# celliern/triflow

Measured on AMD Instinct MI355X. Metric: implicit time-steps/s, 1e6-node 3-var system (member-steps/s over all GPUs), higher is better.
Workload: dtype f64; 1 GPU; BASELINE config 3: M3_film, N=1000000 nodes, periodic, fixed dt=0.001, ROS2; members_per_gpu=1, parallelism=ensemble members sharded by rank, no data-path collective

## Files before the change

__graft_entry__.py:

```python
import os
import sys

ROOT = os.path.dirname(os.path.abspath(__file__))
if ROOT not in sys.path:
    sys.path.insert(0, ROOT)

PREBUILT = ["M1_advdiff", "M2_diff", "M3_film", "M5_stiff"]


def build():
    from triflow_amd import compilers, workloads
    from triflow_amd.model import Model
    compilers.build_runtime_library()
    for name in PREBUILT:
        model = Model(*workloads.model_args(name), hold_compilation=True)
        for seg in (4, 8):
            compilers.build_code_object(model, 0, seg=seg)
    import triflow_amd


def smoke():
    import numpy as np
    from triflow_amd import Model, schemes, workloads
    from oracle import numpy_path as ora
    name, fd, pars, dt, _ = workloads.config_inputs(3, 4096)
    model = Model(*workloads.model_args(name))
    ref = Model(*workloads.model_args(name), compiler=ora.numpy_compiler)
    F = model.F(model.fields_template(**fd), pars)
    Fo = ref.F(ref.fields_template(**fd), pars)
    assert np.array_equal(F, Fo), "F differs from the oracle"
    J = model.J(model.fields_template(**fd), pars)
    Jo = ref.J(ref.fields_template(**fd), pars)
    assert abs(J - Jo).max() <= 4 * np.spacing(abs(Jo).max()), "J differs from the oracle"
    _, new = schemes.ROS2(model)(0.0, model.fields_template(**fd), dt, pars)
    _, new_o = ora.ROS2(ref)(0.0, ref.fields_template(**fd), dt, pars)
    err = np.abs(new.uflat - new_o.uflat).max() / np.abs(new_o.uflat).max()
    assert err < 1e-9, "ROS2 step differs from the oracle: %g" % err
    print("smoke ok: F bit-exact, J <= 4 ulp, ROS2 step rel err %.1e on %s (N=4096)" % (err, name))


if __name__ == "__main__":
    build()
```

triflow_amd/codegen.py:

```python

import ast
import hashlib
import inspect

import numpy as np
from sympy import lambdify

_FUNCS_1 = {"sqrt": "sqrt", "exp": "exp", "log": "log", "sin": "sin", "cos": "cos",
            "tan": "tan", "tanh": "tanh", "sinh": "sinh", "cosh": "cosh",
            "arctan": "atan", "arcsin": "asin", "arccos": "acos",
            "abs": "tf_abs", "absolute": "tf_abs", "fabs": "tf_abs", "sign": "tf_sign",
            "log10": "log10", "log2": "log2", "cbrt": "cbrt", "expm1": "expm1",
            "log1p": "log1p", "floor": "floor", "ceil": "ceil"}


class UnsupportedExpression(NotImplementedError):
    pass


def _dbl(value):
    f = float(value)
    if f != value and not isinstance(value, float):
        raise UnsupportedExpression("integer constant %r is not a double" % (value,))
    if f == int(f) and abs(f) < 2 ** 53:
        return "%d.0" % int(f)
    return f.hex()


class _CEmitter(ast.NodeVisitor):

    def __init__(self, names, uniform_names=()):
        self.names = names
        self.uniform_names = set(uniform_names)
        self.denominators = {}
        self.den_count = {}
        self.shared = {}
        self.host_consts = {}

    def host_const(self, node):
        src = ast.unparse(node)
        k = self.host_consts.setdefault(src, len(self.host_consts))
        return "tf_hc[%d]" % k

    def is_uniform(self, node):
        if isinstance(node, ast.Constant):
            return True
        if isinstance(node, ast.Name):
            return node.id in self.uniform_names or node.id in ("pi", "E", "e")
        if isinstance(node, ast.UnaryOp):
            return self.is_uniform(node.operand)
        if isinstance(node, ast.BinOp):
            return self.is_uniform(node.left) and self.is_uniform(node.right)
        if isinstance(node, ast.Call):
            args = []
            for a in node.args:
                args.extend(a.elts if isinstance(a, (ast.List, ast.Tuple)) else [a])
# ... 85 lines not shown
            for item in items[1:]:
                out = "%s(%s, %s)" % (fn, out, item)
            return out
        if name in ("maximum", "minimum"):
            fn = "tf_max" if name == "maximum" else "tf_min"
            return "%s(%s, %s)" % (fn, self.visit(node.args[0]), self.visit(node.args[1]))
        if name in _FUNCS_1 and len(node.args) == 1:
            if self.is_uniform(node.args[0]) and not isinstance(node.args[0], ast.Constant) \
                    and name not in ("abs", "absolute", "fabs", "sign", "floor", "ceil", "sqrt"):
                return self.host_const(node)
            return "%s(%s)" % (_FUNCS_1[name], self.visit(node.args[0]))
        raise UnsupportedExpression("function %r is not supported by the HIP compiler" % name)

    def generic_visit(self, node):
        raise UnsupportedExpression(ast.dump(node))


def _printed_expressions(symbolic_args, exprs):
    if not exprs:
        return []
    func = lambdify(symbolic_args, exprs, modules=[{"Heaviside": lambda *a: 1}, "numpy"],
                    cse=False)
    src = inspect.getsource(func)
    tree = ast.parse(src)
    fdef = tree.body[0]
    ret = fdef.body[-1]
    if len(fdef.body) != 1 or not isinstance(ret, ast.Return) \
            or not isinstance(ret.value, (ast.List, ast.Tuple)):
        raise UnsupportedExpression("unexpected lambdify output:\n" + src)
    return list(ret.value.elts)


def _c_ident(name):
    return "v_" + "".join(ch if ch.isalnum() else "_" for ch in name)


def _stencil_names(fields, pars, mp, parvec_mask):
    names = {}
    decls = []
    for f, name in enumerate(fields):
        for off in range(-mp, mp + 1):
            key = name if off == 0 else "%s_%s%d" % (name, "m" if off < 0 else "p", abs(off))
            names[key] = _c_ident(key)
            decls.append("const double %s = w[%d][%d];" % (_c_ident(key), f, off + mp))
    for k, name in enumerate(pars):
        names[name] = _c_ident(name)
        decls.append("const double %s = par[%d];" % (_c_ident(name), k))
    names["dx"] = "dx"
    names["x"] = "xc"
    uniform = {"dx"} | {name for k, name in enumerate(pars) if not (parvec_mask >> k) & 1}
    return names, decls, uniform


def lower_model(model, parvec_mask=0, seg=8, sweep_block=64):
    nvar = model._nvar
    fields = list(model._dep_vars) + list(model._help_funcs)
    nh = len(model._help_funcs)
    pars = list(model._pars)
    lo, hi = model._bounds
    mp = (model._window_range - 1) // 2
    if -lo != hi or hi != mp:
        raise UnsupportedExpression("asymmetric stencil window %r" % (model._bounds,))
    if mp < 1:
        mp = 1
    if nvar + nh > 16 or len(pars) > 16:
        raise UnsupportedExpression("too many fields / parameters for the HIP skeleton")
    if mp * nvar > 16:
        raise UnsupportedExpression(
            "the banded solver of the HIP back end handles b = (stencil half width) x (number of dependent "
            "variables) <= 16; this model has b = %d x %d = %d" % (mp, nvar, mp * nvar))
    sparse = [int(k) for k in model._sparse_indices[0]]
    nnz = len(sparse)
    real_mp = (model._window_range - 1) // 2
    pat_eq = [k % nvar for k in sparse]
    pat_var = [(k // nvar) % nvar for k in sparse]
    pat_off = [(k // nvar) // nvar - real_mp for k in sparse]

    names, decls, uniform = _stencil_names(fields, pars, mp, parvec_mask)
    f_nodes = _printed_expressions(model._symbolic_args, model.F_array.tolist())
    j_nodes = _printed_expressions(model._symbolic_args, model._J_sparse_array.tolist())
    host_consts = {}

    def emit_all(nodes):
        first = _CEmitter(names, uniform)
        for n in nodes:
            first.visit(n)
        second = _CEmitter(names, uniform)
        second.shared = first.den_count
        second.host_consts = host_consts
        return second, [second.visit(n) for n in nodes]

    emit_f, f_c = emit_all(f_nodes)
    emit_j, j_c = emit_all(j_nodes)
    uses_x = any("xc" in _tokens(s) for s in f_c + j_c + list(emit_f.denominators) + list(emit_j.denominators))

    j_uniform = [1 if emit_j.is_uniform(n) else 0 for n in j_nodes]

    j_alias, j_alias_scale = _proportional_entries(model, j_uniform)

    def body(outname, exprs, emitter, only=None):
        lines = ["    " + d for d in decls if only is None or d.split("=")[1].strip().startswith("par[")]
        lines += ["    const double* tf_hc = par + %d;" % len(pars)]
        lines += ["    (void)dx; (void)xc; (void)par; (void)tf_hc;"]
        for den, k in sorted(emitter.denominators.items(), key=lambda kv: kv[1]) if only is None else ():
            lines += ["    const double tf_den%d = %s;" % (k, den),
                      "    const double tf_rden%d = 1.0 / tf_den%d;" % (k, k)]
        lines += ["    %s[%d] = %s;" % (outname, i, e) for i, e in enumerate(exprs)
                  if only is None or only[i]]
        return "\n".join(lines)

    def arr(name, values, ctype="int"):
        vals = ", ".join(str(v) for v in values) if values else "0"
        return "static constexpr %s %s[%d] = {%s};" % (ctype, name, max(len(values), 1), vals)

    hc_list = [src_ for src_, _ in sorted(host_consts.items(), key=lambda kv: kv[1])]
    par_is_vec = [1 if (parvec_mask >> k) & 1 else 0 for k in range(len(pars))] + [0] * len(hc_list)
    if len(pars) + len(hc_list) > 16:
        raise UnsupportedExpression("too many parameters + host constants for the HIP skeleton")
    src = "\n".join([
        "// generated by triflow_amd.codegen -- do not edit",
        "// equations: " + " ; ".join(str(e) for e in model._diff_eqs),
        "#define TF_NVAR %d" % nvar,
        "#define TF_NH %d" % nh,
        "#define TF_MP %d" % mp,
        "#define TF_NNZ %d" % nnz,
        "#define TF_NPAR %d" % (len(pars) + len(host_consts)),
        "#define TF_SEG %d" % seg,
        "#define TF_SWEEP_BLOCK %d" % sweep_block,
        "#define TF_USES_X %d" % (1 if uses_x else 0),
        arr("tf_pat_eq", pat_eq), arr("tf_pat_var", pat_var), arr("tf_pat_off", pat_off),
        arr("tf_par_is_vec", par_is_vec, "bool"),
        arr("tf_j_uniform", j_uniform, "bool"),
        arr("tf_j_alias", j_alias), arr("tf_j_alias_scale", [_dbl(v) for v in j_alias_scale], "double"),
        "TF_DEVICE void tf_eval_F(const double (&w)[TF_NVAR + TF_NH][2 * TF_MP + 1], "
        "const double* par, double dx, double xc, double* F) {",
        body("F", f_c, emit_f),
        "}",
        "TF_DEVICE void tf_eval_J(const double (&w)[TF_NVAR + TF_NH][2 * TF_MP + 1], "
        "const double* par, double dx, double xc, double* J) {",
        body("J", j_c, emit_j),
        "}",
        "// the node-independent entries only (tf_j_uniform); same expressions, same bits",
        "TF_DEVICE void tf_eval_J_uniform(const double* par, double dx, double* J) {",
        "    const double xc = 0.0;",
        body("J", j_c, emit_j, only=j_uniform),
        "}",
        ""])
    spec = dict(nvar=nvar, nh=nh, npar=len(pars) + len(hc_list), npar_model=len(pars),
                host_consts=hc_list, mp=mp, nnz=nnz, seg=seg,
                sweep_block=sweep_block, uses_x=int(uses_x), parvec_mask=int(parvec_mask),
                b2=mp * nvar, pat_eq=pat_eq, pat_var=pat_var, pat_off=pat_off, j_uniform=j_uniform,
                j_alias=j_alias, j_alias_scale=j_alias_scale,
                fields=fields, pars=pars)
    return src, spec


PROBE_REDUCTIONS = ("sum", "mean", "integral", "max", "min", "argmax", "argmin")


def _lower_node_expressions(model, exprs, parvec_mask):
    fields = list(model._dep_vars) + list(model._help_funcs)
    pars = list(model._pars)
    mp = max((model._window_range - 1) // 2, 1)
    names, decls, uniform = _stencil_names(fields, pars, mp, parvec_mask)
    import sympy
    for e in exprs:
        if sympy.sympify(e).has(sympy.Heaviside):
            raise UnsupportedExpression("function 'Heaviside' is not supported in a probe or recorder: the HIP "
                                        "compiler takes it as identically one, as the reference does in J; "
                                        "write the step with Max / Min / sign")
    nodes = _printed_expressions(model._symbolic_args, list(exprs))
    first = _CEmitter(names, uniform)
    for n in nodes:
        first.visit(n)
    emit = _CEmitter(names, uniform)
    emit.shared = first.den_count
    out = [emit.visit(n) for n in nodes]
    hc_list = [src_ for src_, _ in sorted(emit.host_consts.items(), key=lambda kv: kv[1])]
    uses_x = any("xc" in _tokens(c) for c in out + list(emit.denominators))
    lines = ["    " + d for d in decls]
    lines += ["    (void)dx; (void)xc; (void)par; (void)tf_hc;"]
    for den, k in sorted(emit.denominators.items(), key=lambda kv: kv[1]):
        lines += ["    const double tf_den%d = %s;" % (k, den),
                  "    const double tf_rden%d = 1.0 / tf_den%d;" % (k, k)]
    return lines, out, hc_list, uses_x, pars


def lower_probes(model, exprs, reductions, parvec_mask=0):
    kinds = [PROBE_REDUCTIONS.index(r) for r in reductions]
    lines, out, hc_list, uses_x, pars = _lower_node_expressions(model, exprs, parvec_mask)
    lines += ["    P[%d] = %s;" % (i, c) for i, c in enumerate(out)]
    block = "\n".join([
        "// device probes, generated by triflow_amd.codegen.lower_probes -- do not edit",
        "// " + " ; ".join("%s: %s" % (r, e) for r, e in zip(reductions, exprs)),
        "#define TF_NPROBE %d" % len(out),
        "#define TF_NPROBE_HC %d" % len(hc_list),
        "#define TF_PROBE_USES_X %d" % (1 if uses_x else 0),
        "static constexpr int tf_probe_kind[%d] = {%s};" % (max(len(kinds), 1),
                                                           ", ".join(map(str, kinds)) or "0"),
        "TF_DEVICE void tf_eval_probe(const double (&w)[TF_NVAR + TF_NH][2 * TF_MP + 1], "
        "const double* par, const double* tf_hc, double dx, double xc, double* P) {",
        "\n".join(lines),
        "}",
        ""])
    spec = dict(nprobe=len(out), kinds=kinds, host_consts=hc_list, pars=pars, uses_x=int(uses_x))
    return block, spec
# ... 169 lines not shown
```

triflow_amd/csrc/tf_kernels.h:

```cpp
#pragma once
#include "tf_args.h"

#ifndef TF_DEVICE
#error "define TF_DEVICE (e.g. __device__ __forceinline__) before including tf_kernels.h"
#endif

#define TF_W (2 * TF_MP + 1)
#define TF_NF (TF_NVAR + TF_NH)
#define TF_B2 (TF_MP * TF_NVAR)

#include "tf_math.h"

#if defined(TF_STAMPS) && defined(__HIP_DEVICE_COMPILE__)
#define TF_STAMP(a, i) do { if ((a).stamps && blockIdx.x == gridDim.x / 2 && threadIdx.x == 0) \
        (a).stamps[i] = __builtin_amdgcn_s_memtime(); } while (0)
#define TF_STAMP_T(a, i, tid) do { if ((a).stamps && blockIdx.x == gridDim.x / 2 && blockIdx.y == 0 && threadIdx.x == (tid)) \
        (a).stamps[i] = __builtin_amdgcn_s_memtime(); } while (0)
#define TF_STAMP_REAL(a, i) do { if ((a).stamps && blockIdx.x == gridDim.x / 2 && threadIdx.x == 0) \
        (a).stamps[i] = __builtin_amdgcn_s_memrealtime(); } while (0)
#define TF_STAMP_IF(a, i, cond) do { if ((a).stamps && (cond) && threadIdx.x == 0) (a).stamps[i] = __builtin_amdgcn_s_memtime(); } while (0)
#define TF_STAMP_REAL_IF(a, i, cond) do { if ((a).stamps && (cond) && threadIdx.x == 0) (a).stamps[i] = __builtin_amdgcn_s_memrealtime(); } while (0)
#define TF_COUNT(a, i) do { if ((a).stamps && (threadIdx.x & 63) == 0) atomicAdd(&(a).stamps[i], 1ull); } while (0)
#define TF_STAMP_L1(a, dir, i) do { if ((dir) > 0 && blockIdx.y == 0) TF_STAMP(a, i); } while (0)
#define TF_WGTRACE(a, k, which) do { if ((a).stamps && threadIdx.x == 0 && blockIdx.y * gridDim.x + blockIdx.x < 1024) \
// ... 437 lines not shown
        const int64_t i = q / L.P, p = q - i * L.P;
        const int64_t s = (int64_t)v * L.plane + i * L.Ptot + (int64_t)e * L.P + p;
        const double d = a.a[s] - a.b[s];
        if (a.ord == 2) acc = tf_fma(d, d, acc);
        else { const double m = tf_abs(d); acc = (m > acc || m != m) ? m : acc; }
    }
    return acc;
}

TF_DEVICE void tfk_dirichlet_elem(const TfDirichletArgs& a, int t) {
    const TfLayout& L = a.L;
    if (t >= a.n * L.nsys) return;
    const int k = t % a.n, e = t / a.n;
    int g = a.node[k];
    if (g < 0) g += L.N;
    int p, i;
    tf_locate(L, g, p, i);
    a.fields[(int64_t)a.var[k] * L.plane + tf_idx(L, e * L.P + p, i)] = a.value[k];
}

TF_DEVICE void tfk_poke_elem(const TfPokeArgs& a, int t) {
    const TfLayout& L = a.L;
    if (t >= a.n * L.nsys) return;
    const int k = t % a.n, e = t / a.n;
    int g = 0, v = 0;
    double val = 0.0;
#pragma unroll
    for (int q = 0; q < TF_POKE_MAX; ++q)
        if (q == k) { g = a.node[q]; v = a.var[q]; val = a.value[q]; }
    if (g < 0) g += L.N;
    int p, i;
    tf_locate(L, g, p, i);
    a.fields[(int64_t)v * L.plane + tf_idx(L, e * L.P + p, i)] = val;
}


template <int B> struct TfBlk { double v[B][B]; };
template <int V> struct TfInt { static constexpr int value = V; };

template <int B>
TF_DEVICE void tf_blk_zero(double (&a)[B][B]) {
#pragma unroll
    for (int r = 0; r < B; ++r)
#pragma unroll
        for (int c = 0; c < B; ++c) a[r][c] = 0.0;
}
template <int B>
TF_DEVICE void tf_blk_copy(double (&d)[B][B], const double (&s)[B][B]) {
#pragma unroll
    for (int r = 0; r < B; ++r)
#pragma unroll
        for (int c = 0; c < B; ++c) d[r][c] = s[r][c];
}
template <int B>
TF_DEVICE void tf_mm_sub(double (&C)[B][B], const double (&A)[B][B], const double (&Bm)[B][B]) {
#pragma unroll
    for (int r = 0; r < B; ++r)
#pragma unroll
        for (int c = 0; c < B; ++c) {
            double acc = C[r][c];
#pragma unroll
            for (int k = 0; k < B; ++k) acc = tf_fma(-A[r][k], Bm[k][c], acc);
            C[r][c] = acc;
        }
}
template <int B>
TF_DEVICE void tf_mm(double (&C)[B][B], const double (&A)[B][B], const double (&Bm)[B][B]) {
#pragma unroll
    for (int r = 0; r < B; ++r)
#pragma unroll
        for (int c = 0; c < B; ++c) {
            double acc = 0.0;
#pragma unroll
            for (int k = 0; k < B; ++k) acc = tf_fma(A[r][k], Bm[k][c], acc);
            C[r][c] = acc;
        }
}
template <int B>
TF_DEVICE void tf_mv_sub(double (&y)[B], const double (&A)[B][B], const double (&x)[B]) {
#pragma unroll
    for (int r = 0; r < B; ++r) {
        double acc = y[r];
#pragma unroll
        for (int k = 0; k < B; ++k) acc = tf_fma(-A[r][k], x[k], acc);
        y[r] = acc;
    }
}
template <int B>
TF_DEVICE void tf_mv(double (&y)[B], const double (&A)[B][B], const double (&x)[B]) {
#pragma unroll
    for (int r = 0; r < B; ++r) {
        double acc = 0.0;
#pragma unroll
        for (int k = 0; k < B; ++k) acc = tf_fma(A[r][k], x[k], acc);
        y[r] = acc;
    }
}

template <int B>
TF_DEVICE bool tf_blk_inverse(const double (&A)[B][B], double (&inv)[B][B]) {
    double a[B][B];
    tf_blk_copy<B>(a, A);
#pragma unroll
    for (int r = 0; r < B; ++r)
#pragma unroll
        for (int c = 0; c < B; ++c) inv[r][c] = (r == c) ? 1.0 : 0.0;
    bool ok = true;
#pragma unroll
    for (int k = 0; k < B; ++k) {
#pragma unroll
        for (int r = k + 1; r < B; ++r) {
            const bool sw = tf_abs(a[r][k]) > tf_abs(a[k][k]);
#pragma unroll
            for (int c = 0; c < B; ++c) {
                const double t0 = a[k][c], t1 = a[r][c];
                a[k][c] = sw ? t1 : t0;
                a[r][c] = sw ? t0 : t1;
                const double u0 = inv[k][c], u1 = inv[r][c];
                inv[k][c] = sw ? u1 : u0;
                inv[r][c] = sw ? u0 : u1;
            }
        }
        const double piv = a[k][k];
        ok = ok && (piv != 0.0) && tf_finite(piv);
        const double rp = 1.0 / piv;
#pragma unroll
        for (int c = 0; c < B; ++c) { a[k][c] *= rp; inv[k][c] *= rp; }
#pragma unroll
        for (int r = 0; r < B; ++r) {
            if (r == k) continue;
            const double f = a[r][k];
#pragma unroll
            for (int c = 0; c < B; ++c) {
                a[r][c] = tf_fma(-f, a[k][c], a[r][c]);
                inv[r][c] = tf_fma(-f, inv[k][c], inv[r][c]);
            }
        }
    }
    return ok;
}

template <int B, int MP> struct TfTips {
    static constexpr int NY = MP * B;
    static constexpr int NV = MP * MP * B * B;
    static constexpr int SIZE = NY + 2 * NV;
    TF_DEVICE_M static int y(int k, int r) { return k * B + r; }
    TF_DEVICE_M static int V(int k, int t, int r, int c) { return NY + ((k * MP + t) * B + r) * B + c; }
    TF_DEVICE_M static int W(int k, int t, int r, int c) { return NY + NV + ((k * MP + t) * B + r) * B + c; }
};


struct TfRowsL1 {
    static constexpr int B = TF_NVAR;
    static constexpr int MP = TF_MP;
    static constexpr bool PIVOT = TF_NVAR == 1;
    const TfLevelArgs& a;
    int pg, e, p, len, start;
    TfJUniform ju;
    TF_DEVICE_M TfRowsL1(const TfLevelArgs& a_, int pg_) : a(a_), pg(pg_) {
        e = pg / a.L.P; p = pg - e * a.L.P;
        len = tf_len(a.L, p); start = tf_start(a.L, p);
        ju.init(a.parsca, a.dx, a.L.nsys, e);
    }
    struct Raw { double jv[TF_NNZ > 0 ? TF_NNZ : 1]; };
    TF_DEVICE_M void request(int i, Raw& r) const {
        const unsigned off = tf_off8(a.L, pg, i);
#pragma unroll
        for (int k = 0; k < TF_NNZ; ++k)
            r.jv[k] = TF_JU(k) ? ju.v[k] : (TF_JA(k) ? 0.0 : tf_ldp(a.Jv, k, a.L.plane, off));
    }
    TF_DEVICE_M void decode(int i, const Raw& raw, double (&row)[2 * TF_MP + 1][TF_NVAR][TF_NVAR]) const {
#pragma unroll
        for (int d = 0; d < TF_W; ++d) tf_blk_zero<TF_NVAR>(row[d]);
#pragma unroll
        for (int k = 0; k < TF_NNZ; ++k) {
            const double jv = TF_JA(k) ? tf_j_alias_scale[k] * raw.jv[tf_j_alias[k] >= 0 ? tf_j_alias[k] : 0] : raw.jv[k];
            row[tf_pat_off[k] + TF_MP][tf_pat_eq[k]][tf_pat_var[k]] = -a.c * jv;
        }
        if (!a.L.periodic) {
            const int gl = start + i, gr = a.L.N - 1 - gl;
            if (gl < TF_MP) {
#pragma unroll
                for (int d = -TF_MP; d < 0; ++d)
                    if (d < -gl) {
#pragma unroll
                        for (int t = -TF_MP + 1; t <= 0; ++t)
                            if (t == -gl) {
#pragma unroll
                                for (int r = 0; r < TF_NVAR; ++r)
#pragma unroll
                                    for (int c = 0; c < TF_NVAR; ++c) {
                                        row[t + TF_MP][r][c] += row[d + TF_MP][r][c];
                                        row[d + TF_MP][r][c] = 0.0;
                                    }
                            }
                    }
            }
            if (gr < TF_MP) {
#pragma unroll
                for (int d = TF_MP; d > 0; --d)
                    if (d > gr) {
#pragma unroll
                        for (int t = TF_MP - 1; t >= 0; --t)
                            if (t == gr) {
#pragma unroll
                                for (int r = 0; r < TF_NVAR; ++r)
#pragma unroll
                                    for (int c = 0; c < TF_NVAR; ++c) {
                                        row[t + TF_MP][r][c] += row[d + TF_MP][r][c];
                                        row[d + TF_MP][r][c] = 0.0;
                                    }
                            }
                    }
            }
        }
#pragma unroll
        for (int r = 0; r < TF_NVAR; ++r) row[TF_MP][r][r] += 1.0;
    }
    TF_DEVICE_M void load(int i, double (&row)[2 * TF_MP + 1][TF_NVAR][TF_NVAR]) const {
        Raw raw;
        request(i, raw);
        decode(i, raw, row);
    }
};

template <int BB>
struct TfRowsBT {
    static constexpr int B = BB;
    static constexpr int MP = 1;
    static constexpr bool PIVOT = false;
    const TfLevelArgs& a;
    int pg, e, p, len, start;
    TF_DEVICE_M TfRowsBT(const TfLevelArgs& a_, int pg_) : a(a_), pg(pg_) {
        e = pg / a.L.P; p = pg - e * a.L.P;
        len = tf_len(a.L, p); start = tf_start(a.L, p);
    }
    struct Raw { double blk[3][BB][BB]; };
    TF_DEVICE_M void request(int i, Raw& r) const {
        const int64_t s = tf_idx(a.L, pg, i);
#pragma unroll
        for (int d = 0; d < 3; ++d)
#pragma unroll
            for (int rr = 0; rr < BB; ++rr)
#pragma unroll
                for (int c = 0; c < BB; ++c)
                    r.blk[d][rr][c] = a.Ablk[(int64_t)((d * BB + rr) * BB + c) * a.L.plane + s];
    }
    TF_DEVICE_M void decode(int i, const Raw& raw, double (&row)[3][BB][BB]) const {
#pragma unroll
        for (int d = 0; d < 3; ++d) tf_blk_copy<BB>(row[d], raw.blk[d]);
        if (!a.L.periodic) {
            const int g = start + i;
            if (g == 0) tf_blk_zero<BB>(row[0]);
            if (g == a.L.N - 1) tf_blk_zero<BB>(row[2]);
        }
    }
    TF_DEVICE_M void load(int i, double (&row)[3][BB][BB]) const {
        Raw raw;
        request(i, raw);
        decode(i, raw, row);
    }
};

#define TF_PIN_REQUESTS() asm volatile("" ::: "memory")
#ifndef TF_BACKSUB_DEPTH
#define TF_BACKSUB_DEPTH 3
#endif
constexpr int tf_ring_depth(int nd, int other = 40) {
    return TF_BACKSUB_DEPTH * nd + other <= 240 ? TF_BACKSUB_DEPTH
         : (2 * nd + other <= 240 && TF_BACKSUB_DEPTH >= 2 ? 2 : 1);
}

template <int B, int MP>
TF_DEVICE int tf_twist_h(int mI, int enabled) {
    return (enabled && MP * B <= 6 && mI >= 4 * MP) ? (mI + 1) / 2 : mI;
}

template <class Rows, int DIR, bool MATRIX, bool DO_V = true, bool DO_W = true, bool DO_G = true>
TF_DEVICE void tf_asm_side(const TfLevelArgs& a, const Rows& own, int pg,
                           const double (&yN)[Rows::MP][Rows::B],
                           const double (&VN)[MATRIX ? Rows::MP : 1][MATRIX ? Rows::MP : 1][Rows::B][Rows::B],
                           const double (&WN)[MATRIX ? Rows::MP : 1][MATRIX ? Rows::MP : 1][Rows::B][Rows::B],
                           double* stage, int* rec) {
    constexpr int B = Rows::B, MP = Rows::MP, W = 2 * MP + 1, BB = MP * B;
    constexpr int VBLK = DIR > 0 ? 0 : 1, WBLK = 1 - VBLK;
    const TfLayout& L = a.L;
    const int e = own.e, p = own.p;
    const bool has = DIR > 0 || L.periodic || p > 0;
    const int ps = DIR > 0 ? p : (p > 0 ? p - 1 : L.P - 1);
    const int r_next = has ? e * a.Lnext.N + ps : -1;
    if (rec) *rec = r_next;
    if (!has) return;
    const int pgs = e * L.P + ps;
    Rows rs(a, pgs);
    const int mIs = rs.len - MP;
#pragma unroll
    for (int t = 0; t < MP; ++t) {
        double row[W][B][B];
        rs.load(mIs + t, row);
        double AV[MP][B][B], AW[MP][B][B], g[B];
#pragma unroll
        for (int t2 = 0; t2 < MP; ++t2) { tf_blk_zero<B>(AV[t2]); tf_blk_zero<B>(AW[t2]); }
        const int64_t s = tf_idx(L, pgs, mIs + t);
#pragma unroll
        for (int r = 0; r < B; ++r) g[r] = (DO_G && DIR > 0 && a.rhs) ? a.rhs[(int64_t)r * L.plane + s] : 0.0;
#pragma unroll
        for (int d = -MP; d <= MP; ++d) {
            const int cn = t + d;
            const bool tip = DIR > 0 ? cn < 0 : cn >= MP;
            const int kt = DIR > 0 ? cn + MP : cn - MP;
            if (DIR > 0 && cn >= 0 && cn < MP) {
                if (MATRIX && DO_W) {
#pragma unroll
                    for (int r = 0; r < B; ++r)
#pragma unroll
// ... 214 lines not shown
#pragma unroll
    for (int d = 0; d < PD; ++d) request(d, pre[d]);
    auto fetch = [&](int q, int jl) {
        install(q, jl, pre[0]);
#pragma unroll
        for (int d = 0; d + 1 < PD; ++d) pre[d] = pre[d + 1];
        request(jl + PD, pre[PD - 1]);
        TF_PIN_REQUESTS();
    };

#pragma unroll
    for (int q = 0; q < MP; ++q) fetch(q, q);
    TF_STAMP_L1(a, DIR, SB + 1);

    auto pivot = [&](int j, auto hist_tag) {
        constexpr int HIST = decltype(hist_tag)::value;
        double Un[UW][B][B], yn[B];
        double En[SPIKE ? MP : 1][B][B];
        if (PIV) {
            fetch(MP, j + MP);
#pragma unroll
            for (int q = 1; q <= MP; ++q) {
                const bool sw = tf_abs(R[q][0][0][0]) > tf_abs(R[0][0][0][0]);
#pragma unroll
                for (int c = 0; c < W; ++c) {
                    const double u = R[0][c][0][0], v = R[q][c][0][0];
                    R[0][c][0][0] = sw ? v : u; R[q][c][0][0] = sw ? u : v;
                }
                { const double u = y[0][0], v = y[q][0]; y[0][0] = sw ? v : u; y[q][0] = sw ? u : v; }
                if (ES) {
#pragma unroll
                    for (int t = 0; t < MP; ++t) {
                        const double u = Es[0][ES ? t : 0][0][0], v = Es[ES ? q : 0][ES ? t : 0][0][0];
                        Es[0][ES ? t : 0][0][0] = sw ? v : u; Es[ES ? q : 0][ES ? t : 0][0][0] = sw ? u : v;
                    }
                }
            }
        }
        {
            double Dinv[B][B];
            ok = tf_blk_inverse<B>(R[0][0], Dinv) && ok;
#pragma unroll
            for (int c = 1; c <= UW; ++c) tf_mm<B>(Un[c - 1], Dinv, R[0][c]);
            tf_mv<B>(yn, Dinv, y[0]);
            if (ES) {
#pragma unroll
                for (int t = 0; t < MP; ++t) tf_mm<B>(En[t], Dinv, Es[0][ES ? t : 0]);
            }
            if (ROLE == 1) {
                double* slot = xch + (j & 1) * (NX * 64);
#pragma unroll
                for (int r = 0; r < B; ++r)
#pragma unroll
                    for (int k = 0; k < B; ++k) slot[(r * B + k) * 64] = Dinv[r][k];
            }
        }
        if (!PIV) fetch(MP, j + MP);
        if (ROLE == 1) {
            double* slot = xch + (j & 1) * (NX * 64);
#pragma unroll
            for (int q = 1; q <= MP; ++q)
#pragma unroll
                for (int r = 0; r < B; ++r)
#pragma unroll
                    for (int k = 0; k < B; ++k) slot[((q * B + r) * B + k) * 64] = R[q][0][r][k];
            TF_WG_BARRIER();
        }
#pragma unroll
        for (int q = 1; q <= MP; ++q) {
#pragma unroll
            for (int c = 1; c <= UW; ++c) tf_mm_sub<B>(R[q][c], R[q][0], Un[c - 1]);
            tf_mv_sub<B>(y[q], R[q][0], yn);
            if (ES) {
#pragma unroll
                for (int t = 0; t < MP; ++t) tf_mm_sub<B>(Es[ES ? q : 0][ES ? t : 0], R[q][0], En[ES ? t : 0]);
            }
        }
        const bool keep = KNOWN || !a.respike;
        const bool keep_u = a.respike ? (DIR > 0 ? j < hdn : j < mI - hdn) : DIR > 0;
        if (STORE_U || STORE_Y) {
            const unsigned off = tf_off8(L, pg, node(j));
            if (STORE_U && keep_u) {
#pragma unroll
                for (int c = 0; c < UW; ++c)
#pragma unroll
                    for (int r = 0; r < B; ++r)
#pragma unroll
                        for (int k = 0; k < B; ++k) {
                            tf_stp(a.Ut, (c * B + r) * B + k, L.plane, off, Un[c][r][k]);
                            if (ES && keep && c < MP)
                                tf_stp(a.Et, (c * B + r) * B + k, L.plane, off, En[ES && c < MP ? c : 0][r][k]);
                        }
            }
            if (STORE_Y && keep) {
                if (KNOWN && YLDS) {
#pragma unroll
                    for (int r = 0; r < B; ++r) ylds[(j * B + r) * 64] = yn[r];
                } else {
#pragma unroll
                    for (int r = 0; r < B; ++r) tf_stp(a.yt, r, L.plane, off, yn[r]);
                }
            }
        }
        if (HIST >= 0) {
            constexpr int H = HIST >= 0 ? HIST : 0;
#pragma unroll
            for (int c = 0; c < UW; ++c) tf_blk_copy<B>(Uh[H][c], Un[c]);
#pragma unroll
            for (int r = 0; r < B; ++r) yh[H][r] = yn[r];
            if (ES) {
#pragma unroll
                for (int t = 0; t < MP; ++t) tf_blk_copy<B>(Eh[ES ? H : 0][ES ? t : 0], En[ES ? t : 0]);
            }
        }
#pragma unroll
        for (int q = 0; q < MP; ++q) {
#pragma unroll
            for (int c = 0; c < W - 1; ++c) tf_blk_copy<B>(R[q][c], R[q + 1][c + 1]);
            tf_blk_zero<B>(R[q][W - 1]);
#pragma unroll
            for (int r = 0; r < B; ++r) y[q][r] = y[q + 1][r];
            if (ES) {
#pragma unroll
                for (int t = 0; t < MP; ++t) tf_blk_copy<B>(Es[ES ? q : 0][ES ? t : 0], Es[ES ? q + 1 : 0][ES ? t : 0]);
            }
        }
    };
    if (KNOWN) {
        const int np = DIR > 0 ? hdn : mI - hdn;
        for (int j = 0; j < np; ++j) {
            if (j == 4) TF_STAMP_L1(a, DIR, SB + 4);
            if (j == 5) TF_STAMP_L1(a, DIR, SB + 5);
            pivot(j, TfInt<-1>());
        }
        TF_STAMP_L1(a, DIR, SB + 2);
        if (!ok) *a.status = 1;
        return;
    }
    for (int j = 0; j < mI - MP; ++j) {
        if (j == 4) TF_STAMP_L1(a, DIR, SB + 4);
        if (j == 5) TF_STAMP_L1(a, DIR, SB + 5);
        pivot(j, TfInt<-1>());
    }
    TF_STAMP_L1(a, DIR, SB + 2);
    pivot(mI - MP, TfInt<0>());
    if (MP > 1) pivot(mI - MP + 1, TfInt<(MP > 1 ? 1 : 0)>());
    static_assert(MP <= 2, "tip epilogue is written for MP <= 2");
    if (ROLE == 1) {
        double* hand = xch + (mI & 1) * (NX * 64);
#pragma unroll
        for (int k = 0; k + 1 < MP; ++k)
#pragma unroll
            for (int r = 0; r < B; ++r)
#pragma unroll
                for (int c = 0; c < B; ++c) hand[((k * B + r) * B + c) * 64] = Uh[k][0][r][c];
        TF_WG_BARRIER();
        TF_WG_BARRIER();
    }
    tf_tips_out<Rows, DIR, SPIKE, ES, true, ROLE == 0>(a, rows, pg, Uh, yh, Eh, asm_stage, asm_rec);
    TF_STAMP_L1(a, DIR, SB + 3);
    if (!ok) *a.status = 1;
}

template <class Rows, int DIR, bool STORE_U, bool STORE_Y>
TF_DEVICE void tfk_rhs_follow_body(const TfLevelArgs& a, int pg, double* xch, double* asm_stage) {
    constexpr int B = Rows::B, MP = Rows::MP, W = 2 * MP + 1;
    constexpr int NX = (1 + MP) * B * B;
    const TfLayout& L = a.L;
    if (pg >= L.Ptot) return;
    if (DIR > 0) TF_STAMP_T(a, 30, 64);
    Rows rows(a, pg);
    const int mI = rows.len - MP;
    auto node = [&](int j) { return DIR > 0 ? j : mI - 1 - j; };
    double Es[MP + 1][MP][B][B], Eh[MP][MP][B][B], y[MP + 1][B], yh[MP][B], ypre[B];
    auto request = [&](int jl) {
#pragma unroll
        for (int r = 0; r < B; ++r)
            ypre[r] = (a.rhs && jl < mI) ? tf_ldp(a.rhs, r, L.plane, tf_off8(L, pg, node(jl < mI ? jl : 0))) : 0.0;
    };
#pragma unroll
    for (int q = 0; q <= MP; ++q) {
#pragma unroll
        for (int t = 0; t < MP; ++t) tf_blk_zero<B>(Es[q][t]);
#pragma unroll
        for (int r = 0; r < B; ++r) y[q][r] = 0.0;
    }
    request(0);
#pragma unroll
    for (int jl = 0; jl < MP; ++jl) {
#pragma unroll
        for (int r = 0; r < B; ++r) y[jl][r] = ypre[r];
        request(jl + 1);
        if (jl < mI) {
            double row[W][B][B];
            rows.load(node(jl), row);
#pragma unroll
            for (int d = -MP; d <= MP; ++d) {
                const int t = MP + jl + d;
                if (jl + d < 0 && t >= 0 && t < MP) tf_blk_copy<B>(Es[jl][t], row[(DIR > 0 ? d : -d) + MP]);
            }
        }
    }
    const int hdn = tf_twist_h<B, MP>(mI, a.twist);
    auto step = [&](int j, auto hist_tag) {
        constexpr int HIST = decltype(hist_tag)::value;
        TF_WG_BARRIER();
        const double* slot = xch + (j & 1) * (NX * 64);
        double Dinv[B][B], En[MP][B][B], yn[B];
#pragma unroll
        for (int r = 0; r < B; ++r)
#pragma unroll
            for (int k = 0; k < B; ++k) Dinv[r][k] = slot[(r * B + k) * 64];
        tf_mv<B>(yn, Dinv, y[0]);
#pragma unroll
        for (int t = 0; t < MP; ++t) tf_mm<B>(En[t], Dinv, Es[0][t]);
#pragma unroll
        for (int r = 0; r < B; ++r) y[MP][r] = ypre[r];
        request(j + MP + 1);
        TF_PIN_REQUESTS();
#pragma unroll
        for (int q = 1; q <= MP; ++q) {
            double M[B][B];
#pragma unroll
            for (int r = 0; r < B; ++r)
#pragma unroll
                for (int k = 0; k < B; ++k) M[r][k] = slot[((q * B + r) * B + k) * 64];
            tf_mv_sub<B>(y[q], M, yn);
#pragma unroll
            for (int t = 0; t < MP; ++t) tf_mm_sub<B>(Es[q][t], M, En[t]);
        }
        const bool keep_u = a.respike ? (DIR > 0 ? j < hdn : j < mI - hdn) : DIR > 0;
        if ((STORE_U || STORE_Y) && !a.respike) {
            const unsigned off = tf_off8(L, pg, node(j));
            if (STORE_U && keep_u) {
#pragma unroll
                for (int c = 0; c < MP; ++c)
#pragma unroll
                    for (int r = 0; r < B; ++r)
#pragma unroll
                        for (int k = 0; k < B; ++k) tf_stp(a.Et, (c * B + r) * B + k, L.plane, off, En[c][r][k]);
            }
            if (STORE_Y) {
#pragma unroll
                for (int r = 0; r < B; ++r) tf_stp(a.yt, r, L.plane, off, yn[r]);
            }
        }
        if (HIST >= 0) {
            constexpr int H = HIST >= 0 ? HIST : 0;
#pragma unroll
            for (int t = 0; t < MP; ++t) tf_blk_copy<B>(Eh[H][t], En[t]);
#pragma unroll
            for (int r = 0; r < B; ++r) yh[H][r] = yn[r];
        }
#pragma unroll
        for (int q = 0; q < MP; ++q) {
#pragma unroll
            for (int t = 0; t < MP; ++t) tf_blk_copy<B>(Es[q][t], Es[q + 1][t]);
#pragma unroll
            for (int r = 0; r < B; ++r) y[q][r] = y[q + 1][r];
        }
#pragma unroll
        for (int t = 0; t < MP; ++t) tf_blk_zero<B>(Es[MP][t]);
    };
    if (DIR > 0) TF_STAMP_T(a, 31, 64);
    for (int j = 0; j < mI - MP; ++j) step(j, TfInt<-1>());
    step(mI - MP, TfInt<0>());
    if (MP > 1) step(mI - MP + 1, TfInt<(MP > 1 ? 1 : 0)>());
    if (DIR > 0) TF_STAMP_T(a, 32, 64);
    double Uh[MP][1][B][B];
#pragma unroll
    for (int k = 0; k < MP; ++k) tf_blk_zero<B>(Uh[k][0]);
    TF_WG_BARRIER();
    const double* hand = xch + (mI & 1) * (NX * 64);
#pragma unroll
    for (int k = 0; k + 1 < MP; ++k)
#pragma unroll
        for (int r = 0; r < B; ++r)
#pragma unroll
            for (int c = 0; c < B; ++c) Uh[k][0][r][c] = hand[((k * B + r) * B + c) * 64];
    TF_WG_BARRIER();
    if (DIR > 0) TF_STAMP_T(a, 33, 64);
    tf_tips_out<Rows, DIR, true, true, false, true>(a, rows, pg, Uh, yh, Eh, asm_stage, nullptr);
    if (DIR > 0) TF_STAMP_T(a, 34, 64);
}

template <int BB>
TF_DEVICE void tfk_bt_lu_body(const TfLevelArgs& a, int pg, int dir) {
    typedef TfTips<BB, 1> Tip;
    const TfLayout& L = a.L;
    if (pg >= L.Ptot) return;
    TfRowsBT<BB> rows(a, pg);
    const int mI = rows.len - 1;
    const int di = dir > 0 ? 0 : 1;
    bool ok = true;
    double S[BB][BB], Un[BB][BB];
    for (int j = 0; j < mI; ++j) {
        const int i = dir > 0 ? j : mI - 1 - j;
        const int64_t s = tf_idx(L, pg, i);
        double row[3][BB][BB];
        rows.load(i, row);
        tf_blk_copy<BB>(S, row[1]);
        if (j > 0) tf_mm_sub<BB>(S, row[dir > 0 ? 0 : 2], Un);
        double Dinv[BB][BB];
        ok = tf_blk_inverse<BB>(S, Dinv) && ok;
        tf_mm<BB>(Un, Dinv, row[dir > 0 ? 2 : 0]);
        double* Uout = dir > 0 ? a.Ut : a.Unup;
#pragma unroll
        for (int r = 0; r < BB; ++r)
#pragma unroll
            for (int c = 0; c < BB; ++c) {
                a.Dinv[(int64_t)((di * BB + r) * BB + c) * L.plane + s] = Dinv[r][c];
                Uout[(int64_t)(r * BB + c) * L.plane + s] = Un[r][c];
            }
    }
    double* tips = dir > 0 ? a.tips_dn : a.tips_up;
#pragma unroll
    for (int r = 0; r < BB; ++r)
#pragma unroll
        for (int c = 0; c < BB; ++c)
            tips[(int64_t)(dir > 0 ? Tip::W(0, 0, r, c) : Tip::V(0, 0, r, c)) * L.Ptot + pg] = Un[r][c];
    if (!ok) *a.status = 1;
}

template <int BB>
TF_DEVICE void tfk_bt_col_body(const TfLevelArgs& a, int pg, int dir, int col) {
    typedef TfTips<BB, 1> Tip;
    const TfLayout& L = a.L;
    if (pg >= L.Ptot) return;
    const int e = pg / L.P, p = pg - e * L.P;
    const int len = tf_len(L, p), mI = len - 1, start = tf_start(L, p);
    const int di = dir > 0 ? 0 : 1;
    const bool is_rhs = col >= BB;
// ... 165 lines not shown
                        }
                    }
        }
    }
}

template <class Rows, bool WITH_E = true>
TF_DEVICE void tfk_backsub_body(const TfLevelArgs& a, int pg) {
    constexpr int B = Rows::B, MP = Rows::MP;
    constexpr int UW = Rows::PIVOT ? 2 * MP : MP;
    const TfLayout& L = a.L;
    if (pg >= L.Ptot) return;
    const int e = pg / L.P, p = pg - e * L.P;
    const int len = tf_len(L, p), mI = len - MP;
    const bool has_above = L.periodic || p > 0;
    const int pa = p > 0 ? p - 1 : L.P - 1;
    double sa[MP][B], xn[UW][B];
#pragma unroll
    for (int t = MP; t < UW; ++t)
#pragma unroll
        for (int r = 0; r < B; ++r) xn[t][r] = 0.0;
    {
        int p2, i2;
        tf_locate(a.Lnext, p, p2, i2);
        const int64_t s2 = tf_idx(a.Lnext, e * a.Lnext.P + p2, i2);
#pragma unroll
        for (int t = 0; t < MP; ++t)
#pragma unroll
            for (int r = 0; r < B; ++r) xn[t][r] = a.xnext[tf_next_x(a, e, p, s2, t * B + r, MP * B)];
        tf_locate(a.Lnext, pa, p2, i2);
        const int64_t s2a = tf_idx(a.Lnext, e * a.Lnext.P + p2, i2);
#pragma unroll
        for (int t = 0; t < MP; ++t)
#pragma unroll
            for (int r = 0; r < B; ++r) sa[t][r] = has_above ? a.xnext[tf_next_x(a, e, pa, s2a, t * B + r, MP * B)] : 0.0;
    }
#pragma unroll
    for (int t = 0; t < MP; ++t) {
        const int64_t s = tf_idx(L, pg, mI + t);
#pragma unroll
        for (int r = 0; r < B; ++r) a.x[(int64_t)r * L.plane + s] = xn[t][r];
    }
    struct Node { double y[B]; double U[UW][B][B]; double E[WITH_E ? MP : 1][B][B]; };
    auto load = [&](int j, Node& n) {
        const unsigned off = tf_off8(L, pg, j);
#pragma unroll
        for (int r = 0; r < B; ++r) n.y[r] = tf_ldp(a.yt, r, L.plane, off);
#pragma unroll
        for (int c = 0; c < UW; ++c)
#pragma unroll
            for (int r = 0; r < B; ++r)
#pragma unroll
                for (int k = 0; k < B; ++k) {
                    n.U[c][r][k] = tf_ldp(a.Ut, (c * B + r) * B + k, L.plane, off);
                    if (WITH_E && c < MP) n.E[WITH_E && c < MP ? c : 0][r][k] = tf_ldp(a.Et, (c * B + r) * B + k, L.plane, off);
                }
    };
    constexpr int D = tf_ring_depth(B + UW * B * B + (WITH_E ? MP * B * B : 0));
    Node ring[D];
#pragma unroll
    for (int d = 0; d < D; ++d)
        if (mI - 1 - d >= 0) load(mI - 1 - d, ring[d]);
    for (int j0 = mI - 1; j0 >= 0; j0 -= D) {
#pragma unroll
        for (int d = 0; d < D; ++d) {
            const int j = j0 - d;
            if (j < 0) break;
            const Node& cur = ring[d];
            const int64_t s = tf_idx(L, pg, j);
            double x[B];
#pragma unroll
            for (int r = 0; r < B; ++r) x[r] = cur.y[r];
#pragma unroll
            for (int c = 0; c < UW; ++c) tf_mv_sub<B>(x, cur.U[c], xn[c]);
            if (WITH_E) {
#pragma unroll
                for (int c = 0; c < MP; ++c) tf_mv_sub<B>(x, cur.E[WITH_E ? c : 0], sa[c]);
            }
#pragma unroll
            for (int c = UW - 1; c > 0; --c)
#pragma unroll
                for (int r = 0; r < B; ++r) xn[c][r] = xn[c - 1][r];
#pragma unroll
            for (int r = 0; r < B; ++r) { xn[0][r] = x[r]; a.x[(int64_t)r * L.plane + s] = x[r]; }
            if (j - D >= 0) load(j - D, ring[d]);
        }
    }
}

template <int n>
TF_DEVICE bool tf_dense_solve(double (&S)[n][n], double (&g)[n]) {
    bool ok = true;
#pragma unroll
    for (int k = 0; k < n; ++k) {
#pragma unroll
        for (int r = k + 1; r < n; ++r) {
            const bool sw = tf_abs(S[r][k]) > tf_abs(S[k][k]);
#pragma unroll
            for (int c = k; c < n; ++c) { const double u = S[k][c], v = S[r][c]; S[k][c] = sw ? v : u; S[r][c] = sw ? u : v; }
            { const double u = g[k], v = g[r]; g[k] = sw ? v : u; g[r] = sw ? u : v; }
        }
        const double piv = S[k][k];
        ok = ok && (piv != 0.0) && (piv == piv);
        const double rp = 1.0 / piv;
#pragma unroll
        for (int c = k + 1; c < n; ++c) S[k][c] = S[k][c] * rp;
        g[k] = g[k] * rp;
#pragma unroll
        for (int r = k + 1; r < n; ++r) {
            const double f = S[r][k];
#pragma unroll
            for (int c = k + 1; c < n; ++c) S[r][c] = tf_fma(-f, S[k][c], S[r][c]);
            g[r] = tf_fma(-f, g[k], g[r]);
        }
    }
#pragma unroll
    for (int k = n - 2; k >= 0; --k)
#pragma unroll
        for (int c = k + 1; c < n; ++c) g[k] = tf_fma(-S[k][c], g[c], g[k]);
    return ok;
}

template <class Rows, bool YLDS = false>
TF_DEVICE void tfk_backsub_twist_body(const TfLevelArgs& a, int pg, int dir,
                                      const double* ylds_dn = nullptr, const double* ylds_up = nullptr) {
    constexpr int B = Rows::B, MP = Rows::MP, NB = MP * B;
    static_assert(!Rows::PIVOT, "the re-elimination form is for block sizes that do not exchange rows");
    const TfLayout& L = a.L;
    if (pg >= L.Ptot) return;
    const int e = pg / L.P, p = pg - e * L.P;
    const int len = tf_len(L, p), mI = len - MP;
    const int h = tf_twist_h<B, MP>(mI, a.twist), hu = mI - h;
    if (dir == 1 && hu == 0) return;
    double xn[MP][B];
    const int jstart = hu == 0 ? mI - 1 : (dir == 0 ? h - MP - 1 : hu - MP - 1);
    auto nat = [&](int j) { return dir == 0 ? j : mI - 1 - j; };
    auto ldU = [&](int node_nat, double (&U)[MP][B][B], double (&y)[B]) {
        const unsigned off = tf_off8(L, pg, node_nat);
        if (YLDS) {
            const double* src = node_nat < h ? ylds_dn + node_nat * B * 64 : ylds_up + (mI - 1 - node_nat) * B * 64;
#pragma unroll
            for (int r = 0; r < B; ++r) y[r] = src[r * 64];
        } else {
#pragma unroll
            for (int r = 0; r < B; ++r) y[r] = tf_ldp(a.yt, r, L.plane, off);
        }
#pragma unroll
        for (int c = 0; c < MP; ++c)
#pragma unroll
            for (int r = 0; r < B; ++r)
#pragma unroll
                for (int k = 0; k < B; ++k) U[c][r][k] = tf_ldp(a.Ut, (c * B + r) * B + k, L.plane, off);
    };
    struct Upd { double b[B], k[B]; };
    const bool upd = YLDS && a.upd_n > 0;
    auto upd_load = [&](int nd, Upd& u) {
        if (upd) {
            const unsigned off = tf_off8(L, pg, nd);
#pragma unroll
            for (int r = 0; r < B; ++r) {
                u.b[r] = tf_ldp(a.upd_base, r, L.plane, off);
                u.k[r] = a.upd_n > 1 ? tf_ldp(a.upd_k0, r, L.plane, off) : 0.0;
            }
        }
    };
    auto emit = [&](int nd, const double (&x)[B], const Upd& u) {
        const int64_t s = tf_idx(L, pg, nd);
        if (upd) {
#pragma unroll
            for (int r = 0; r < B; ++r) {
                double acc;
                if (a.upd_n > 1) { acc = a.upd_c0 * u.k[r]; acc = acc + a.upd_c1 * x[r]; }
                else acc = a.upd_c0 * x[r];
                a.upd_out[(int64_t)r * L.plane + s] = u.b[r] + acc;
            }
        } else {
#pragma unroll
            for (int r = 0; r < B; ++r) a.x[(int64_t)r * L.plane + s] = x[r];
        }
    };
    double xsep[MP][B], xmid[MP][B];
    const bool own_sep = hu == 0 || dir == 0;
    if (own_sep) {
        int p2, i2;
        tf_locate(a.Lnext, p, p2, i2);
        const int64_t s2 = tf_idx(a.Lnext, e * a.Lnext.P + p2, i2);
#pragma unroll
        for (int t = 0; t < MP; ++t) {
#pragma unroll
            for (int r = 0; r < B; ++r) {
                const double v = a.xnext[tf_next_x(a, e, p, s2, t * B + r, MP * B)];
                xn[t][r] = v;
                xsep[t][r] = v;
            }
        }
    }
    struct Node { double y[B]; double U[MP][B][B]; Upd u; };
    auto load = [&](int j, Node& n) { ldU(nat(j), n.U, n.y); upd_load(nat(j), n.u); };
    constexpr int D = tf_ring_depth(3 * B + MP * B * B, 2 * (MP * B) * (MP * B) + 2 * MP * B + MP * B * B + B);
    Node ring[D];
#pragma unroll
    for (int d = 0; d < D; ++d)
        if (jstart - d >= 0) load(jstart - d, ring[d]);
    if (hu != 0) {
        double Tc[NB][NB], Tg[NB];
// ... 216 lines not shown
```

Before: 2413 steps/s.

## Exploit block sparsity of solver blocks via compile-time nonzero mask

Computes a structural nonzero mask for the per-node variable blocks (Jacobian pattern closed under fill-in) and emits it into the generated header. The block matmul, matvec and inverse routines, plus the loads and stores of U, E, Dinv and handoff blocks, skip entries that are structurally zero. This cuts FLOPs and memory traffic in the banded block solver for models whose variable coupling is not dense, at the cost of an extra code path and a reliance on the fill-in closure being correct. The pivot-swap logic is restricted to rows that share structure, which changes pivoting behaviour slightly.

```diff
diff --git a/__graft_entry__.py b/__graft_entry__.py
--- a/__graft_entry__.py
+++ b/__graft_entry__.py
@@ -6,6 +6,7 @@
     sys.path.insert(0, ROOT)
 
 PREBUILT = ["M1_advdiff", "M2_diff", "M3_film", "M5_stiff"]
+PREBUILT_DENSE = ["M3_film", "M5_stiff"]
 
 
 def build():
@@ -16,6 +17,17 @@
         model = Model(*workloads.model_args(name), hold_compilation=True)
         for seg in (4, 8):
             compilers.build_code_object(model, 0, seg=seg)
+    saved = os.environ.get("TRIFLOW_BLOCK_MASK")
+    os.environ["TRIFLOW_BLOCK_MASK"] = "0"
+    try:
+        for name in PREBUILT_DENSE:
+            model = Model(*workloads.model_args(name), hold_compilation=True)
+            compilers.build_code_object(model, 0, seg=4)
+    finally:
+        if saved is None:
+            del os.environ["TRIFLOW_BLOCK_MASK"]
+        else:
+            os.environ["TRIFLOW_BLOCK_MASK"] = saved
     import triflow_amd
 
 
diff --git a/triflow_amd/codegen.py b/triflow_amd/codegen.py
--- a/triflow_amd/codegen.py
+++ b/triflow_amd/codegen.py
@@ -2,6 +2,7 @@
 import ast
 import hashlib
 import inspect
+import os
 
 import numpy as np
 from sympy import lambdify
@@ -193,6 +194,21 @@
     return names, decls, uniform
 
 
+def block_mask(nvar, pat_eq, pat_var):
+    if os.environ.get("TRIFLOW_BLOCK_MASK", "1") == "0":
+        return [[True] * nvar for _ in range(nvar)]
+    m = [[r == c for c in range(nvar)] for r in range(nvar)]
+    for e, v in zip(pat_eq, pat_var):
+        m[e][v] = True
+    for k in range(nvar):
+        for r in range(nvar):
+            if m[r][k]:
+                for c in range(nvar):
+                    if m[k][c]:
+                        m[r][c] = True
+    return m
+
+
 def lower_model(model, parvec_mask=0, seg=8, sweep_block=64):
     nvar = model._nvar
     fields = list(model._dep_vars) + list(model._help_funcs)
@@ -254,6 +270,8 @@
         vals = ", ".join(str(v) for v in values) if values else "0"
         return "static constexpr %s %s[%d] = {%s};" % (ctype, name, max(len(values), 1), vals)
 
+    blk_nz = block_mask(nvar, pat_eq, pat_var)
+    blk_full = all(all(row) for row in blk_nz)
     hc_list = [src_ for src_, _ in sorted(host_consts.items(), key=lambda kv: kv[1])]
     par_is_vec = [1 if (parvec_mask >> k) & 1 else 0 for k in range(len(pars))] + [0] * len(hc_list)
     if len(pars) + len(hc_list) > 16:
@@ -270,6 +288,10 @@
         "#define TF_SWEEP_BLOCK %d" % sweep_block,
         "#define TF_USES_X %d" % (1 if uses_x else 0),
         arr("tf_pat_eq", pat_eq), arr("tf_pat_var", pat_var), arr("tf_pat_off", pat_off),
+        "// entries of a solver block that can be non-zero (block_mask): [equation][variable]",
+        "#define TF_BLK_FULL %d" % (1 if blk_full else 0),
+        "static constexpr bool tf_blk_nz[%d][%d] = {%s};" % (
+            nvar, nvar, ", ".join("{%s}" % ", ".join("true" if v else "false" for v in row) for row in blk_nz)),
         arr("tf_par_is_vec", par_is_vec, "bool"),
         arr("tf_j_uniform", j_uniform, "bool"),
         arr("tf_j_alias", j_alias), arr("tf_j_alias_scale", [_dbl(v) for v in j_alias_scale], "double"),
@@ -292,7 +314,7 @@
                 sweep_block=sweep_block, uses_x=int(uses_x), parvec_mask=int(parvec_mask),
                 b2=mp * nvar, pat_eq=pat_eq, pat_var=pat_var, pat_off=pat_off, j_uniform=j_uniform,
                 j_alias=j_alias, j_alias_scale=j_alias_scale,
-                fields=fields, pars=pars)
+                blk_nz=blk_nz, fields=fields, pars=pars)
     return src, spec
 
 
diff --git a/triflow_amd/csrc/tf_kernels.h b/triflow_amd/csrc/tf_kernels.h
--- a/triflow_amd/csrc/tf_kernels.h
+++ b/triflow_amd/csrc/tf_kernels.h
@@ -513,67 +513,94 @@
 #pragma unroll
         for (int c = 0; c < B; ++c) d[r][c] = s[r][c];
 }
+template <int B> struct TfMask {
+    static constexpr bool FULL = true;
+    TF_DEVICE_M static constexpr bool nz(int, int) { return true; }
+    TF_DEVICE_M static constexpr bool same(int, int) { return true; }
+};
+#if defined(TF_BLK_FULL) && !TF_BLK_FULL
+template <> struct TfMask<TF_NVAR> {
+    static constexpr bool FULL = false;
+    TF_DEVICE_M static constexpr bool nz(int r, int c) { return tf_blk_nz[r][c]; }
+    TF_DEVICE_M static constexpr bool same(int r, int c) { return tf_blk_nz[r][c] && tf_blk_nz[c][r]; }
+};
+#endif
+
 template <int B>
 TF_DEVICE void tf_mm_sub(double (&C)[B][B], const double (&A)[B][B], const double (&Bm)[B][B]) {
+    typedef TfMask<B> M;
 #pragma unroll
     for (int r = 0; r < B; ++r)
 #pragma unroll
         for (int c = 0; c < B; ++c) {
+            if (!M::nz(r, c)) { C[r][c] = 0.0; continue; }
             double acc = C[r][c];
 #pragma unroll
-            for (int k = 0; k < B; ++k) acc = tf_fma(-A[r][k], Bm[k][c], acc);
+            for (int k = 0; k < B; ++k)
+                if (M::nz(r, k) && M::nz(k, c)) acc = tf_fma(-A[r][k], Bm[k][c], acc);
             C[r][c] = acc;
         }
 }
 template <int B>
 TF_DEVICE void tf_mm(double (&C)[B][B], const double (&A)[B][B], const double (&Bm)[B][B]) {
+    typedef TfMask<B> M;
 #pragma unroll
     for (int r = 0; r < B; ++r)
 #pragma unroll
         for (int c = 0; c < B; ++c) {
             double acc = 0.0;
 #pragma unroll
-            for (int k = 0; k < B; ++k) acc = tf_fma(A[r][k], Bm[k][c], acc);
+            for (int k = 0; k < B; ++k)
+                if (M::nz(r, c) && M::nz(r, k) && M::nz(k, c)) acc = tf_fma(A[r][k], Bm[k][c], acc);
             C[r][c] = acc;
         }
 }
 template <int B>
 TF_DEVICE void tf_mv_sub(double (&y)[B], const double (&A)[B][B], const double (&x)[B]) {
+    typedef TfMask<B> M;
 #pragma unroll
     for (int r = 0; r < B; ++r) {
         double acc = y[r];
 #pragma unroll
-        for (int k = 0; k < B; ++k) acc = tf_fma(-A[r][k], x[k], acc);
+        for (int k = 0; k < B; ++k)
+            if (M::nz(r, k)) acc = tf_fma(-A[r][k], x[k], acc);
         y[r] = acc;
     }
 }
 template <int B>
 TF_DEVICE void tf_mv(double (&y)[B], const double (&A)[B][B], const double (&x)[B]) {
+    typedef TfMask<B> M;
 #pragma unroll
     for (int r = 0; r < B; ++r) {
         double acc = 0.0;
 #pragma unroll
-        for (int k = 0; k < B; ++k) acc = tf_fma(A[r][k], x[k], acc);
+        for (int k = 0; k < B; ++k)
+            if (M::nz(r, k)) acc = tf_fma(A[r][k], x[k], acc);
         y[r] = acc;
     }
 }
 
 template <int B>
 TF_DEVICE bool tf_blk_inverse(const double (&A)[B][B], double (&inv)[B][B]) {
+    typedef TfMask<B> M;
     double a[B][B];
-    tf_blk_copy<B>(a, A);
 #pragma unroll
     for (int r = 0; r < B; ++r)
 #pragma unroll
-        for (int c = 0; c < B; ++c) inv[r][c] = (r == c) ? 1.0 : 0.0;
+        for (int c = 0; c < B; ++c) {
+            a[r][c] = M::nz(r, c) ? A[r][c] : 0.0;
+            inv[r][c] = (r == c) ? 1.0 : 0.0;
+        }
     bool ok = true;
 #pragma unroll
     for (int k = 0; k < B; ++k) {
 #pragma unroll
         for (int r = k + 1; r < B; ++r) {
+            if (!M::same(r, k)) continue;
             const bool sw = tf_abs(a[r][k]) > tf_abs(a[k][k]);
 #pragma unroll
             for (int c = 0; c < B; ++c) {
+                if (!M::nz(k, c)) continue;
                 const double t0 = a[k][c], t1 = a[r][c];
                 a[k][c] = sw ? t1 : t0;
                 a[r][c] = sw ? t0 : t1;
@@ -586,13 +613,15 @@
         ok = ok && (piv != 0.0) && tf_finite(piv);
         const double rp = 1.0 / piv;
 #pragma unroll
-        for (int c = 0; c < B; ++c) { a[k][c] *= rp; inv[k][c] *= rp; }
+        for (int c = 0; c < B; ++c)
+            if (M::nz(k, c)) { a[k][c] *= rp; inv[k][c] *= rp; }
 #pragma unroll
         for (int r = 0; r < B; ++r) {
-            if (r == k) continue;
+            if (r == k || !M::nz(r, k)) continue;
             const double f = a[r][k];
 #pragma unroll
             for (int c = 0; c < B; ++c) {
+                if (!M::nz(k, c)) continue;
                 a[r][c] = tf_fma(-f, a[k][c], a[r][c]);
                 inv[r][c] = tf_fma(-f, inv[k][c], inv[r][c]);
             }
@@ -615,6 +644,7 @@
     static constexpr int B = TF_NVAR;
     static constexpr int MP = TF_MP;
     static constexpr bool PIVOT = TF_NVAR == 1;
+    static constexpr bool MASKED = true;
     const TfLevelArgs& a;
     int pg, e, p, len, start;
     TfJUniform ju;
@@ -690,6 +720,7 @@
     static constexpr int B = BB;
     static constexpr int MP = 1;
     static constexpr bool PIVOT = false;
+    static constexpr bool MASKED = false;
     const TfLevelArgs& a;
     int pg, e, p, len, start;
     TF_DEVICE_M TfRowsBT(const TfLevelArgs& a_, int pg_) : a(a_), pg(pg_) {
@@ -722,6 +753,9 @@
         decode(i, raw, row);
     }
 };
+
+template <class Rows>
+TF_DEVICE_M constexpr bool tf_kept(int r, int k) { return !Rows::MASKED || TfMask<Rows::B>::nz(r, k); }
 
 #define TF_PIN_REQUESTS() asm volatile("" ::: "memory")
 #ifndef TF_BACKSUB_DEPTH
@@ -1042,7 +1076,8 @@
 #pragma unroll
                 for (int r = 0; r < B; ++r)
 #pragma unroll
-                    for (int k = 0; k < B; ++k) slot[(r * B + k) * 64] = Dinv[r][k];
+                    for (int k = 0; k < B; ++k)
+                        if (tf_kept<Rows>(r, k)) slot[(r * B + k) * 64] = Dinv[r][k];
             }
         }
         if (!PIV) fetch(MP, j + MP);
@@ -1053,7 +1088,8 @@
 #pragma unroll
                 for (int r = 0; r < B; ++r)
 #pragma unroll
-                    for (int k = 0; k < B; ++k) slot[((q * B + r) * B + k) * 64] = R[q][0][r][k];
+                    for (int k = 0; k < B; ++k)
+                        if (tf_kept<Rows>(r, k)) slot[((q * B + r) * B + k) * 64] = R[q][0][r][k];
             TF_WG_BARRIER();
         }
 #pragma unroll
@@ -1077,6 +1113,7 @@
                     for (int r = 0; r < B; ++r)
 #pragma unroll
                         for (int k = 0; k < B; ++k) {
+                            if (!tf_kept<Rows>(r, k)) continue;
                             tf_stp(a.Ut, (c * B + r) * B + k, L.plane, off, Un[c][r][k]);
                             if (ES && keep && c < MP)
                                 tf_stp(a.Et, (c * B + r) * B + k, L.plane, off, En[ES && c < MP ? c : 0][r][k]);
@@ -1143,7 +1180,8 @@
 #pragma unroll
             for (int r = 0; r < B; ++r)
 #pragma unroll
-                for (int c = 0; c < B; ++c) hand[((k * B + r) * B + c) * 64] = Uh[k][0][r][c];
+                for (int c = 0; c < B; ++c)
+                    if (tf_kept<Rows>(r, c)) hand[((k * B + r) * B + c) * 64] = Uh[k][0][r][c];
         TF_WG_BARRIER();
         TF_WG_BARRIER();
     }
@@ -1200,7 +1238,7 @@
 #pragma unroll
         for (int r = 0; r < B; ++r)
 #pragma unroll
-            for (int k = 0; k < B; ++k) Dinv[r][k] = slot[(r * B + k) * 64];
+            for (int k = 0; k < B; ++k) Dinv[r][k] = tf_kept<Rows>(r, k) ? slot[(r * B + k) * 64] : 0.0;
         tf_mv<B>(yn, Dinv, y[0]);
 #pragma unroll
         for (int t = 0; t < MP; ++t) tf_mm<B>(En[t], Dinv, Es[0][t]);
@@ -1214,7 +1252,7 @@
 #pragma unroll
             for (int r = 0; r < B; ++r)
 #pragma unroll
-                for (int k = 0; k < B; ++k) M[r][k] = slot[((q * B + r) * B + k) * 64];
+                for (int k = 0; k < B; ++k) M[r][k] = tf_kept<Rows>(r, k) ? slot[((q * B + r) * B + k) * 64] : 0.0;
             tf_mv_sub<B>(y[q], M, yn);
 #pragma unroll
             for (int t = 0; t < MP; ++t) tf_mm_sub<B>(Es[q][t], M, En[t]);
@@ -1228,7 +1266,8 @@
 #pragma unroll
                     for (int r = 0; r < B; ++r)
 #pragma unroll
-                        for (int k = 0; k < B; ++k) tf_stp(a.Et, (c * B + r) * B + k, L.plane, off, En[c][r][k]);
+                        for (int k = 0; k < B; ++k)
+                            if (tf_kept<Rows>(r, k)) tf_stp(a.Et, (c * B + r) * B + k, L.plane, off, En[c][r][k]);
             }
             if (STORE_Y) {
 #pragma unroll
@@ -1267,7 +1306,7 @@
 #pragma unroll
         for (int r = 0; r < B; ++r)
 #pragma unroll
-            for (int c = 0; c < B; ++c) Uh[k][0][r][c] = hand[((k * B + r) * B + c) * 64];
+            for (int c = 0; c < B; ++c) Uh[k][0][r][c] = tf_kept<Rows>(r, c) ? hand[((k * B + r) * B + c) * 64] : 0.0;
     TF_WG_BARRIER();
     if (DIR > 0) TF_STAMP_T(a, 33, 64);
     tf_tips_out<Rows, DIR, true, true, false, true>(a, rows, pg, Uh, yh, Eh, asm_stage, nullptr);
@@ -1539,8 +1578,9 @@
             for (int r = 0; r < B; ++r)
 #pragma unroll
                 for (int k = 0; k < B; ++k) {
-                    n.U[c][r][k] = tf_ldp(a.Ut, (c * B + r) * B + k, L.plane, off);
-                    if (WITH_E && c < MP) n.E[WITH_E && c < MP ? c : 0][r][k] = tf_ldp(a.Et, (c * B + r) * B + k, L.plane, off);
+                    const bool kept = tf_kept<Rows>(r, k);
+                    n.U[c][r][k] = kept ? tf_ldp(a.Ut, (c * B + r) * B + k, L.plane, off) : 0.0;
+                    if (WITH_E && c < MP) n.E[WITH_E && c < MP ? c : 0][r][k] = kept ? tf_ldp(a.Et, (c * B + r) * B + k, L.plane, off) : 0.0;
                 }
     };
     constexpr int D = tf_ring_depth(B + UW * B * B + (WITH_E ? MP * B * B : 0));
@@ -1637,7 +1677,8 @@
 #pragma unroll
             for (int r = 0; r < B; ++r)
 #pragma unroll
-                for (int k = 0; k < B; ++k) U[c][r][k] = tf_ldp(a.Ut, (c * B + r) * B + k, L.plane, off);
+                for (int k = 0; k < B; ++k)
+                    U[c][r][k] = tf_kept<Rows>(r, k) ? tf_ldp(a.Ut, (c * B + r) * B + k, L.plane, off) : 0.0;
     };
     struct Upd { double b[B], k[B]; };
     const bool upd = YLDS && a.upd_n > 0;
```

Result: faster. 2676 steps/s, median of 6 (+10.9%).
